# xianlopez/optical_flow

Measured on AMD Instinct MI355X. Metric: image-pairs/sec training, 384x512 batch=8 per GPU, higher is better.
Workload: dtype fp32

## Files before the change

optical_flow_amd/csrc/conv_f32.hip:

```cpp
#include "common.h"
#include "conv_dev.h"
#include "conv_narrow.h"

#include <algorithm>

namespace oflow {

template <int BM, int BN, int WAVES_M, int WAVES_N, int MODE>
__global__ __launch_bounds__(256, 2) void conv_gemm_f32(GemmArgs a) {
  constexpr int WM = BM / WAVES_M, WN = BN / WAVES_N;
  constexpr int TM = WM / 32, TN = WN / 32;
  static_assert(WAVES_M * WAVES_N == 4, "4 waves");
  static_assert(TM >= 1 && TN >= 1 && WM % 32 == 0 && WN % 32 == 0, "tile");
  constexpr bool A_KCONTIG = (MODE != MODE_WGRAD);
  constexpr int SA = BM + 4;
  constexpr int SB = BN + 4;
  constexpr int A_SLOTS = BM * BK / 4 / 256;
  constexpr int B_QUADS = BK * BN / 4;
  constexpr int B_SLOTS = (B_QUADS + 255) / 256;
  static_assert(A_SLOTS >= 1, "BM >= 64");

  static_assert(2 * BK * (SA + SB) >= 4 * 1024, "epilogue images fit LDS");
  __shared__ float smem[2 * BK * (SA + SB)];
  float (*As)[BK * SA] = reinterpret_cast<float (*)[BK * SA]>(smem);
// ... 2669 lines not shown
    }
  };
  auto store_halo = [&](int hb) {
#pragma unroll
    for (int k = 0; k < SW_HQ; ++k) {
      const int q = tid + NT * k;
      if (q >= SW_HH * SW_HX) continue;
      const int hy = q / SW_HX, hx = q - hy * SW_HX;
      float* dst = Hs[hb] + hy * 8 * SW_HC + (hx & 1) * SW_HC + (hx >> 1);
      dst[0] = hv[k].x;
      dst[2 * SW_HC] = hv[k].y;
      dst[4 * SW_HC] = hv[k].z;
      dst[6 * SW_HC] = hv[k].w;
    }
  };

  f32x4 acc[2][4];
#pragma unroll
  for (int i = 0; i < 2; ++i)
#pragma unroll
    for (int j = 0; j < 4; ++j)
#pragma unroll
      for (int r = 0; r < 4; ++r) acc[i][j][r] = 0.f;
  const int l16 = lane & 15, kg = lane >> 4;
  int a_off[2];
#pragma unroll
  for (int mt = 0; mt < 2; ++mt) {
    const int m = min(16 * (2 * wave + mt) + l16, 146);
    const int tap = m / 3, ci = m - 3 * tap, r = tap / 7, sc = tap - 7 * r;
    a_off[mt] = (r * 8 + ci * 2 + (sc & 1)) * SW_HC + 8 * kg + (sc >> 1);
  }

  if (nchunks > 0) {
    load_halo(t_begin);
    load_dz(0, dv[0], 0);
    if (nchunks > 1) load_dz(1, dv[1], 1);
    store_halo(0);
  }
  auto chunk = [&](int c, float* dvc, int set) {
    const int j = c % SW_TH, tl = c / SW_TH;
    const int buf = c & 1;
    if (j == 0 && tl + 1 < ntiles) load_halo(t_begin + tl + 1);
    if constexpr (FUSED) {
      if (tid < 256) form_dz(set, (j & 1) != 0, dvc);
    }
    store_dz(buf, dvc);
    __syncthreads();
    if (c + 2 < nchunks) load_dz(c + 2, dvc, set);
    if (j == 1 && tl + 1 < ntiles) store_halo((tl + 1) & 1);
    const float* hrow = Hs[tl & 1] + 2 * j * 8 * SW_HC;
    bf16x8 av[2][NP];
#pragma unroll
    for (int mt = 0; mt < 2; ++mt) {
      float v[8];
#pragma unroll
      for (int e = 0; e < 8; ++e) v[e] = hrow[a_off[mt] + e];
      if (NP == 1)
        av[mt][0] = __builtin_bit_cast(bf16x8, pack_bf16x8(make_float4(v[0], v[1], v[2], v[3]),
                                                           make_float4(v[4], v[5], v[6], v[7])));
      else
        split3x8(v, av[mt][0], av[mt][NP / 2], av[mt][NP - 1]);
    }
#pragma unroll
    for (int nt = 0; nt < 4; ++nt) {
      bf16x8 bv[NP];
#pragma unroll
      for (int p = 0; p < NP; ++p)
        bv[p] = __builtin_bit_cast(bf16x8, Ds[buf][(p * 4 + kg) * 64 + nt * 16 + l16]);
#pragma unroll
      for (int mt = 0; mt < 2; ++mt) {
        f32x4 x = acc[mt][nt];
        if (NP == 3) {
          x = __builtin_amdgcn_mfma_f32_16x16x32_bf16(av[mt][NP - 1], bv[0], x, 0, 0, 0);
          x = __builtin_amdgcn_mfma_f32_16x16x32_bf16(av[mt][0], bv[NP - 1], x, 0, 0, 0);
          x = __builtin_amdgcn_mfma_f32_16x16x32_bf16(av[mt][NP / 2], bv[NP / 2], x, 0, 0, 0);
          x = __builtin_amdgcn_mfma_f32_16x16x32_bf16(av[mt][NP / 2], bv[0], x, 0, 0, 0);
          x = __builtin_amdgcn_mfma_f32_16x16x32_bf16(av[mt][0], bv[NP / 2], x, 0, 0, 0);
        }
        acc[mt][nt] = __builtin_amdgcn_mfma_f32_16x16x32_bf16(av[mt][0], bv[0], x, 0, 0, 0);
      }
    }
  };
  for (int c = 0; c < nchunks; c += 2) {
    chunk(c, dv[0], 0);
    if (c + 1 < nchunks) chunk(c + 1, dv[1], 1);
  }

  float* slab = a.slab + (int64_t)split * a.split_stride;
#pragma unroll
  for (int mt = 0; mt < 2; ++mt)
#pragma unroll
    for (int rr = 0; rr < 4; ++rr) {
      const int m = 16 * (2 * wave + mt) + 4 * kg + rr;
      if (m >= 147) continue;
      const int tap = m / 3, ci = m - 3 * tap;
#pragma unroll
      for (int nt = 0; nt < 4; ++nt) {
        const int co = nt * 16 + l16;
        if (co < a.N) slab[(int64_t)(tap * 4 + ci) * a.slab_ld + co] = acc[mt][nt][rr];
      }
    }
  if (FUSED) {
    float* Cs = reinterpret_cast<float*>(&Ds[0][0]);
    __syncthreads();
    if (tid < 256) {
      Cs[d_kg * 64 + d_co] = f_st;
      Cs[256 + d_kg * 64 + d_co] = f_stz;
    }
    __syncthreads();
    if (tid < 128 && (tid & 63) < a.N) {
      const int o = (tid >> 6) * 256, cc = tid & 63;
      slab[(int64_t)(196 + (tid >> 6)) * a.slab_ld + cc] =
          (Cs[o + cc] + Cs[o + 64 + cc]) + (Cs[o + 128 + cc] + Cs[o + 192 + cc]);
    }
  } else if (a.colsum) {
    float* Cs = reinterpret_cast<float*>(&Ds[0][0]);
    __syncthreads();
    if (tid < 256) Cs[d_kg * 64 + d_co] = csum;
    __syncthreads();
    if (tid < 64 && tid < a.N)
      slab[(int64_t)196 * a.slab_ld + tid] = (Cs[tid] + Cs[64 + tid]) + (Cs[128 + tid] + Cs[192 + tid]);
  }
}

__global__ __launch_bounds__(256) void stem_bn_final(const float* __restrict__ slab, int splits,
                                                     int64_t split_stride, int ld, int c,
                                                     const float* __restrict__ gamma,
                                                     const float* __restrict__ var, float eps,
                                                     float* __restrict__ dgamma,
                                                     float* __restrict__ dbeta,
                                                     float* __restrict__ dbias, int accum) {
  __shared__ float red[2][4][64];
  const int co = threadIdx.x & 63, g = threadIdx.x >> 6;
  const int s0 = (int)((int64_t)g * splits / 4), s1 = (int)((int64_t)(g + 1) * splits / 4);
  float st = 0.f, stz = 0.f;
  if (co < c) {
    for (int sp = s0; sp < s1; ++sp) {
      st += slab[sp * split_stride + 196 * (int64_t)ld + co];
      stz += slab[sp * split_stride + 197 * (int64_t)ld + co];
    }
  }
  red[0][g][co] = st;
  red[1][g][co] = stz;
  __syncthreads();
  if (g != 0 || co >= c) return;
  st = (red[0][0][co] + red[0][1][co]) + (red[0][2][co] + red[0][3][co]);
  stz = (red[1][0][co] + red[1][1][co]) + (red[1][2][co] + red[1][3][co]);
  const float db = st * gamma[co] * rsqrtf(var[co] + eps);
  if (dbeta) dbeta[co] = accum ? dbeta[co] + st : st;
  if (dgamma) dgamma[co] = accum ? dgamma[co] + stz : stz;
  if (dbias) dbias[co] = accum ? dbias[co] + db : db;
}

template <int WAVES_CI, int WAVES_CO, int WAVES_R, int XH>
__global__ __launch_bounds__(64 * WAVES_CI * WAVES_CO * WAVES_R, 1) void conv_wgrad_tile_x3(GemmArgs a) {
  constexpr int NT = 64 * WAVES_CI * WAVES_CO * WAVES_R;
  static_assert(WAVES_R == 3, "one kernel row per wave group");
  constexpr int CIB = 32 * WAVES_CI, COB = 32 * WAVES_CO, KS = 3, HH = XH + KS - 1, NP = 3;
  constexpr int XQ = HH * KS * 2 * (CIB / 4), XS = (XQ + NT - 1) / NT;
  constexpr int PL = KS * HH * CIB * 2;
  __shared__ uint4 Xs[NP * PL];

  auto xrow = [](int ci) { return ci ^ ((ci >> 2) & 2); };
  auto xoct = [](int ci) { return (ci >> 4) & 1; };
  const int tid = threadIdx.x;
  const int lane = tid & 63;
  const int wave = __builtin_amdgcn_readfirstlane(tid >> 6);
  const int wgid = xcd_remap(blockIdx.x, gridDim.x);
  const int split = wgid / a.tiles_total;
  const int tile = wgid - split * a.tiles_total;
  const int tile_co = tile % a.n_tiles;
  const int tile_ci = tile / a.n_tiles;
  const int ci0 = tile_ci * CIB, co0 = tile_co * COB;
  const int t_begin = split * a.k_per_split;
  const int t_end = min(a.K, t_begin + a.k_per_split);
  const int steps = max(0, t_end - t_begin);
  const int tiles_x = (a.wo + TT_W - 1) / TT_W, tiles_y = (a.ho + XH - 1) / XH;
  const rsrc_t rx = make_rsrc(a.A, a.a_bytes);
  const rsrc_t rd = make_rsrc(a.B, a.b_bytes);
  const int wr = wave / (WAVES_CI * WAVES_CO);
  const int wci0 = ((wave / WAVES_CO) % WAVES_CI) * 32;
  const int wco0 = (wave % WAVES_CO) * 32;
  const int lrow = lane & 31, lk = lane >> 5;
  const bool do_colsum = a.colsum && tile_ci == 0 && wci0 == 0 && wr == 0;

  const int xcq = tid % (CIB / 4);
  const bool xc_ok = ci0 + 4 * xcq < a.kc;
  float4 xv[XS][8];
  auto load_x = [&](int t) {
    const int b = t / (tiles_x * tiles_y);
    const int trem = t - b * tiles_x * tiles_y;
    const int oy0 = (trem / tiles_x) * XH, ox0 = (trem % tiles_x) * TT_W;
    const int iy0 = oy0 - a.pt, ix00 = ox0 - a.pl;
#pragma unroll
    for (int j = 0; j < XS; ++j) {
      const int q = tid + NT * j;
      const int r2 = q / (CIB / 4);
      const int half = r2 & 1, s = (r2 >> 1) % KS, hy = (r2 >> 1) / KS;
      const int iy = iy0 + hy;
      const bool rok = q < XQ && xc_ok && (unsigned)iy < (unsigned)a.h;
      const int ix0 = ix00 + 8 * half + s;
      const int base = ((b * a.h + iy) * a.w + ix0) * a.lda + ci0 + 4 * xcq;
#pragma unroll
      for (int e = 0; e < 8; ++e) {
        const bool ok = rok && (unsigned)(ix0 + e) < (unsigned)a.w;
        xv[j][e] = bload4(rx, ok ? (uint32_t)((base + e * a.lda) * 4) : kOOB);
      }
    }
  };
  auto store_x = [&]() {
#pragma unroll
    for (int j = 0; j < XS; ++j) {
      const int q = tid + NT * j;
      if (q < XQ) {
        const int r2 = q / (CIB / 4);
        const int half = r2 & 1, s = (r2 >> 1) % KS, hy = (r2 >> 1) / KS;
        const int ci = 4 * xcq;
        uint4* blk = &Xs[(s * HH + hy) * CIB * 2];
#pragma unroll
        for (int c = 0; c < 4; ++c) {
          float v8[8];
#pragma unroll
          for (int e = 0; e < 8; ++e) v8[e] = (&xv[j][e].x)[c];
          bf16x8 h, m, l;
          split3x8(v8, h, m, l);
          const int idx = xrow(ci + c) * 2 + (half ^ xoct(ci + c));
          blk[idx] = __builtin_bit_cast(uint4, h);
          blk[PL + idx] = __builtin_bit_cast(uint4, m);
          blk[2 * PL + idx] = __builtin_bit_cast(uint4, l);
        }
      }
    }
  };
  const int co = co0 + wco0 + lrow;
  const bool co_ok = co < a.nb;
  const uint32_t dy_lane = (uint32_t)((8 * lk * a.ldb + co) * 4);
  const bool dy_co_full = co0 + COB <= a.nb;
  auto load_dy = [&](float (&dv)[8], int t, int kk) {
    const int b = t / (tiles_x * tiles_y);
    const int trem = t - b * tiles_x * tiles_y;
    const int oy = (trem / tiles_x) * XH + kk, ox0 = (trem % tiles_x) * TT_W;
    if (dy_co_full && oy < a.ho && ox0 + TT_W <= a.wo) {
      const int so = ((b * a.ho + oy) * a.wo + ox0) * a.ldb * 4;
#pragma unroll
      for (int e = 0; e < 8; ++e)
        dv[e] = __builtin_bit_cast(float, __builtin_amdgcn_raw_buffer_load_b32(
                                              rd, dy_lane + e * a.ldb * 4, so, 0));
      return;
    }
    const int ox = ox0 + 8 * lk;
    const bool rok = co_ok && oy < a.ho;
    const int base = ((b * a.ho + oy) * a.wo + ox) * a.ldb + co;
#pragma unroll
    for (int e = 0; e < 8; ++e) {
      const bool ok = rok && ox + e < a.wo;
      dv[e] = bload1(rd, ok ? (uint32_t)((base + e * a.ldb) * 4) : kOOB);
    }
  };

  f32x16 acc[KS];
#pragma unroll
  for (int t = 0; t < KS; ++t)
#pragma unroll
    for (int r = 0; r < 16; ++r) acc[t][r] = 0.f;
  const int a_base = xrow(wci0 + lrow) * 2 + (lk ^ xoct(wci0 + lrow));
  float colacc = 0.f;
  float dcur[8], dnext[8];

  if (steps > 0) {
    load_x(t_begin);
    load_dy(dcur, t_begin, 0);
    store_x();
  }
  __syncthreads();
  for (int i = 0; i < steps; ++i) {
    const int t = t_begin + i;
    const bool more = i + 1 < steps;
    if (more) load_x(t + 1);
#pragma unroll
    for (int kk = 0; kk < XH; ++kk) {
      if (kk + 1 < XH) load_dy(dnext, t, kk + 1);
      else if (more) load_dy(dnext, t + 1, 0);
      __builtin_amdgcn_sched_barrier(0);
      bf16x8 bh, bm, bl;
      split3x8(dcur, bh, bm, bl);
      if (do_colsum) {
#pragma unroll
        for (int e = 0; e < 8; ++e) colacc += dcur[e];
      }
      bf16x8 fa[2][NP];
      auto load_a = [&](bf16x8 (&f)[NP], int s) {
        const int xa = (s * HH + kk + wr) * CIB * 2 + a_base;
#pragma unroll
        for (int p = 0; p < NP; ++p) f[p] = __builtin_bit_cast(bf16x8, Xs[p * PL + xa]);
      };
      load_a(fa[0], 0);
#pragma unroll
      for (int s = 0; s < KS; ++s) {
          if (s + 1 < KS) load_a(fa[(s + 1) & 1], s + 1);
          __builtin_amdgcn_sched_barrier(0);
          const bf16x8 ah = fa[s & 1][0], am = fa[s & 1][1], al = fa[s & 1][2];
          f32x16 x = acc[s];
          x = __builtin_amdgcn_mfma_f32_32x32x16_bf16(al, bh, x, 0, 0, 0);
          x = __builtin_amdgcn_mfma_f32_32x32x16_bf16(ah, bl, x, 0, 0, 0);
          x = __builtin_amdgcn_mfma_f32_32x32x16_bf16(am, bm, x, 0, 0, 0);
          x = __builtin_amdgcn_mfma_f32_32x32x16_bf16(am, bh, x, 0, 0, 0);
          x = __builtin_amdgcn_mfma_f32_32x32x16_bf16(ah, bm, x, 0, 0, 0);
          acc[s] = __builtin_amdgcn_mfma_f32_32x32x16_bf16(ah, bh, x, 0, 0, 0);
          __builtin_amdgcn_sched_barrier(0);
      }
#pragma unroll
      for (int e = 0; e < 8; ++e) dcur[e] = dnext[e];
    }
    __syncthreads();
    if (more) store_x();
    __syncthreads();
  }

  float* S = a.slab + (int64_t)split * a.split_stride;
  if (do_colsum) {
    const float v = colacc + __shfl_xor(colacc, 32);
    if (lk == 0 && co < a.N) S[(int64_t)a.M * a.slab_ld + co] = v;
  }
  if (co < a.N) {
#pragma unroll
    for (int s = 0; s < KS; ++s)
#pragma unroll
      for (int r = 0; r < 16; ++r) {
        const int ci = ci0 + wci0 + (r & 3) + 8 * (r >> 2) + 4 * lk;
        if (ci < a.kc) S[((int64_t)(wr * KS + s) * a.kc + ci) * a.slab_ld + co] = acc[s][r];
      }
  }
}

__device__ __forceinline__ int wgx3b_slot(int ci, int oct) {
  return (ci >> 3) * 16 + ((2 * (ci & 7) + oct) ^ (((ci >> 3) & 3) << 1));
}

template <int CIB>
__device__ __forceinline__ int wgx3b_sw(int hx) {
  return ((hx >> 3) & 1) | (CIB == 64 ? ((hx >> 1) & 1) << 1 : 0);
}

template <int WAVES_CI, int WAVES_CO, int XH, int MI, int NP, int STG>
__device__ __forceinline__ void wgrad_x3b_body(const GemmArgs& a) {
  constexpr int NJ = 2 / MI;
  static_assert(MI * NJ == 2, "18 accumulator tiles per wave");
  static_assert(NP == 1 || NP == 3, "planes");
  static_assert(STG == 0 || STG == 1, "staging: three shifted copies / one pixel-major image");
  constexpr int NT = 64 * WAVES_CI * WAVES_CO;
  constexpr int CIB = 16 * MI * WAVES_CI, COB = 16 * NJ * WAVES_CO, KS = 3, HH = XH + KS - 1;
  static_assert(XH % 2 == 0 && (CIB == 32 || CIB == 64), "k-steps of 2 tile rows; wgx3b_sw");
  constexpr int HW = TT_W + KS - 1;
  constexpr int XQ = STG ? HH * HW * (CIB / 4) : HH * KS * 2 * (CIB / 4), XS = (XQ + NT - 1) / NT;
  constexpr int RB = CIB * 2;
  constexpr int PL = KS * HH * RB;
  constexpr int PXB = CIB * 2;
  constexpr int PLB = HH * HW * PXB, IMGB = NP * PLB;
  constexpr int LDSB = STG ? 2 * IMGB : NP * PL * 16;
  static_assert(NT / 64 * 512 * 4 <= LDSB && LDSB % 16 == 0, "epilogue images fit LDS");
  __shared__ uint4 Xs[LDSB / 16];
  char* const xlds = reinterpret_cast<char*>(Xs);

  const int tid = threadIdx.x;
  const int lane = tid & 63;
  const int wave = __builtin_amdgcn_readfirstlane(tid >> 6);
  const int wgid = xcd_remap(blockIdx.x, gridDim.x);
  const int split = wgid / a.tiles_total;
  const int tile = wgid - split * a.tiles_total;
  const int tile_co = tile % a.n_tiles;
  const int tile_ci = tile / a.n_tiles;
  const int ci0 = tile_ci * CIB, co0 = tile_co * COB;
  const int t_begin = split * a.k_per_split;
  const int t_end = min(a.K, t_begin + a.k_per_split);
  const int steps = max(0, t_end - t_begin);
  const int tiles_x = (a.wo + TT_W - 1) / TT_W, tiles_y = (a.ho + XH - 1) / XH;
  const rsrc_t rx = make_rsrc(a.A, a.a_bytes);
  const rsrc_t rd = make_rsrc(a.B, a.b_bytes);
  const int wci0 = (wave / WAVES_CO) * 16 * MI;
  const int wco0 = (wave % WAVES_CO) * 16 * NJ;
  const int l16 = lane & 15, lq = lane >> 4;

  const int xcq = tid % (CIB / 4);
  const bool xc_ok = ci0 + 4 * xcq < a.kc;
  constexpr int XE = STG ? 1 : 8;
  float4 xv[XS][XE];
  auto load_x = [&](int t) {
    const int b = t / (tiles_x * tiles_y);
    const int trem = t - b * tiles_x * tiles_y;
    const int oy0 = (trem / tiles_x) * XH, ox0 = (trem % tiles_x) * TT_W;
    const int iy0 = oy0 - a.pt, ix00 = ox0 - a.pl;
#pragma unroll
    for (int j = 0; j < XS; ++j) {
      const int q = tid + NT * j;
      if constexpr (STG == 1) {
        const int hp = q / (CIB / 4);
        const int hy = hp / HW, hx = hp - hy * HW;
        const int iy = iy0 + hy, ix = ix00 + hx;
        const bool ok = q < XQ && xc_ok && (unsigned)iy < (unsigned)a.h &&
                        (unsigned)ix < (unsigned)a.w;
        const int base = ((b * a.h + iy) * a.w + ix) * a.lda + ci0 + 4 * xcq;
        xv[j][0] = bload4(rx, ok ? (uint32_t)(base * 4) : kOOB);
      } else {
        const int r2 = q / (CIB / 4);
        const int half = r2 & 1, s = (r2 >> 1) % KS, hy = (r2 >> 1) / KS;
        const int iy = iy0 + hy;
        const bool rok = q < XQ && xc_ok && (unsigned)iy < (unsigned)a.h;
        const int ix0 = ix00 + 8 * half + s;
        const int base = ((b * a.h + iy) * a.w + ix0) * a.lda + ci0 + 4 * xcq;
#pragma unroll
        for (int e = 0; e < 8; ++e) {
          const bool ok = rok && (unsigned)(ix0 + e) < (unsigned)a.w;
          xv[j][e] = bload4(rx, ok ? (uint32_t)((base + e * a.lda) * 4) : kOOB);
        }
      }
    }
  };
  auto store_x = [&](int j, int buf) {
    const int q = tid + NT * j;
    if (XQ % NT == 0 || q < XQ) {
      if constexpr (STG == 1) {
        const int hp = q / (CIB / 4);
        const int hx = hp % HW;
        char* dst = xlds + buf * IMGB + hp * PXB + (((xcq >> 2) ^ wgx3b_sw<CIB>(hx)) << 5) +
                    8 * (xcq & 3);
        if constexpr (NP == 1) {
          *reinterpret_cast<uint2*>(dst) = pack_bf16x4(xv[j][0]);
        } else {
          uint2 h, m, l;
          split3x4(xv[j][0], h, m, l);
          *reinterpret_cast<uint2*>(dst) = h;
          *reinterpret_cast<uint2*>(dst + PLB) = m;
          *reinterpret_cast<uint2*>(dst + 2 * PLB) = l;
        }
      } else {
        const int r2 = q / (CIB / 4);
        const int half = r2 & 1, s = (r2 >> 1) % KS, hy = (r2 >> 1) / KS;
        uint4* blk = &Xs[(s * HH + hy) * RB];
#pragma unroll
        for (int c = 0; c < 4; ++c) {
          float v8[8];
#pragma unroll
          for (int e = 0; e < 8; ++e) v8[e] = (&xv[j][e].x)[c];
          const int idx = wgx3b_slot(4 * xcq + c, half);
          if constexpr (NP == 1) {
            blk[idx] = pack_bf16x8(make_float4(v8[0], v8[1], v8[2], v8[3]),
                                   make_float4(v8[4], v8[5], v8[6], v8[7]));
          } else {
            bf16x8 h, m, l;
            split3x8(v8, h, m, l);
            blk[idx] = __builtin_bit_cast(uint4, h);
            blk[PL + idx] = __builtin_bit_cast(uint4, m);
            blk[2 * PL + idx] = __builtin_bit_cast(uint4, l);
          }
        }
      }
    }
  };
  auto store_x_all = [&](int buf) {
#pragma unroll
    for (int j = 0; j < XS; ++j) store_x(j, buf);
  };
  int co[NJ];
  bool co_ok[NJ];
#pragma unroll
  for (int j = 0; j < NJ; ++j) {
    co[j] = co0 + wco0 + 16 * j + l16;
    co_ok[j] = co[j] < a.nb;
  }
  const int prow = lq >> 1, pcol = 8 * (lq & 1);
  const bool dy_co_full = co0 + COB <= a.nb;
  const uint32_t dy_lane = (uint32_t)(((prow * a.wo + pcol) * a.ldb + co0 + wco0 + l16) * 4);
  auto load_dy = [&](float (&dv)[NJ][8], int t, int kk) {
    const int b = t / (tiles_x * tiles_y);
    const int trem = t - b * tiles_x * tiles_y;
    const int oyr = (trem / tiles_x) * XH + 2 * kk, ox0 = (trem % tiles_x) * TT_W;
    if (dy_co_full && oyr + 1 < a.ho && ox0 + TT_W <= a.wo) {
      const int so = ((b * a.ho + oyr) * a.wo + ox0) * a.ldb * 4;
#pragma unroll
      for (int j = 0; j < NJ; ++j)
#pragma unroll
        for (int e = 0; e < 8; ++e)
          dv[j][e] = __builtin_bit_cast(float, __builtin_amdgcn_raw_buffer_load_b32(
                                                   rd, dy_lane + (e * a.ldb + 16 * j) * 4, so, 0));
      return;
    }
    const int oy = oyr + prow, ox = ox0 + pcol;
    const bool rok = oy < a.ho;
#pragma unroll
    for (int j = 0; j < NJ; ++j) {
      const int base = ((b * a.ho + oy) * a.wo + ox) * a.ldb + co[j];
#pragma unroll
      for (int e = 0; e < 8; ++e) {
        const bool ok = rok && co_ok[j] && ox + e < a.wo;
// ... 1535 lines not shown
  return with_cfg(T[cfg], cfg);
}

bool wgt_ok(const of_conv_desc* d, bool bf16) {
  if (!tile_ok(d)) return false;
  if (bf16) return true;
  const int64_t npix = (int64_t)d->n * d->ho * d->wo;
  return d->cout == 64 || (d->cout % 128 == 0 && npix <= 8 * 96 * 128);
}
int wgt_cfg(const of_conv_desc* d) { return d->cout > 64 ? 0 : 2; }
void wgt_blocks(const of_conv_desc* d, int& cib, int& cob) {
  cib = wgt_cfg(d) == 0 ? 32 : 64;
  cob = wgt_cfg(d) == 0 ? 128 : 64;
}

int wgx3_cfg(const of_conv_desc* d) {
  if (!tile_ok(d)) return -1;
  if (d->cout == 64) return d->cin_p % 64 == 0 || !g_wgx3_c4 ? 2 : 4;
  return d->cout % 128 == 0 ? 0 : d->cout == 96 ? 1 : d->cout == 32 ? 3 : -1;
}
bool wgx3_ok(const of_conv_desc* d) { return wgx3_cfg(d) >= 0; }
void wgx3_blocks(const of_conv_desc* d, int& cib, int& cob) {
  const int c = wgx3_cfg(d);
  cib = c == 2 || c == 3 ? 64 : 32;
  cob = c == 0 ? 128 : c == 1 ? 96 : c == 2 || c == 4 ? 64 : 32;
}

static int g_stem_wg = 1;
bool stem_wg_ok(const of_conv_desc* d) { return g_stem_wg && stem_x3_ok(d) && d->cin == 3; }
int stem_wg_tiles(const of_conv_desc* d) {
  return d->n * (int)cdiv(d->ho, SW_TH) * (int)cdiv(d->wo, SW_TW);
}

static int g_wgrad_wgs = 4;
static int g_x3_direct = 1;
static int g_bnp_b16 = 0;

static int g_gemm_b16 = 6;
static int g_wgt_pf = 1;

enum class Fam { narrow, gemm_f32, gemm_bf16, gemm_x3, gemm_b16, tile_bf16, tile_x3, tile_b16,
                 tile_ws, stem };
enum class WFam { narrow, stem, tile_x3, tile_b16, gemm_x3, gemm_b16, tile, gemm_bf16, gemm_f32 };

Fam gemm_family(int prec, int mode) {
  if (!prec) return Fam::gemm_f32;
  if (prec == 2) return Fam::gemm_x3;
  return (g_gemm_b16 & (mode == MODE_FWD ? 1 : 2)) ? Fam::gemm_b16 : Fam::gemm_bf16;
}
Fam tile_family(const of_conv_desc* d, int prec, int mode, bool bnp = false) {
  if (prec == 2) return Fam::tile_x3;
  if (ws_ok(d, mode)) return Fam::tile_ws;
  return g_tile_b16 == 1 || (bnp && g_bnp_b16) ? Fam::tile_b16 : Fam::tile_bf16;
}
Fam fwd_family(const of_conv_desc* d, int prec, bool plain, bool stem_kernel = true) {
  if (!prec) return narrow_ok(d) && plain ? Fam::narrow : Fam::gemm_f32;
  if (tile_ok(d)) return tile_family(d, prec, MODE_FWD);
  if (stem_kernel && (prec == 2 || g_stem_bf16) && g_stem_x3 && stem_x3_ok(d)) return Fam::stem;
  return gemm_family(prec, MODE_FWD);
}
Fam dgrad_family(const of_conv_desc* d, int prec, bool bnp = false) {
  if (!prec) return narrow_ok(d) ? Fam::narrow : Fam::gemm_f32;
  return tile_ok(d) ? tile_family(d, prec, MODE_DGRAD, bnp) : gemm_family(prec, MODE_DGRAD);
}

GemmArgs plan_args(const of_conv_desc* d, const Geo& g, int mode, Fam f, bool in_place = false) {
  if (f == Fam::tile_bf16 || f == Fam::tile_x3 || f == Fam::tile_b16 || f == Fam::tile_ws)
    return tile_args(d, g, mode, f == Fam::tile_x3, f == Fam::tile_b16, f == Fam::tile_ws);
  const bool k16 = f != Fam::gemm_f32 && f != Fam::narrow;
  GemmArgs a = mode == MODE_FWD ? fwd_args(d, g, k16) : dgrad_args(d, g, k16, in_place);
  if (f == Fam::gemm_x3 || f == Fam::gemm_b16) gemm_x3_plan(a);
  return a;
}

template <int MODE>
int launch_family(Fam f, const GemmArgs& a, hipStream_t s, double flops) {
  switch (f) {
    case Fam::tile_x3: return launch<MODE>(tile_x3_launch<MODE>(a), a, s, flops);
    case Fam::tile_ws:
      return launch<MODE>(with_cfg(tile_ws_launch(a, MODE), kind(KIND_TILE_WS, MODE, 0)), a, s, flops);
    case Fam::tile_b16: return launch<MODE>(tile_b16_launch<MODE>(a), a, s, flops);
    case Fam::tile_bf16: return launch<MODE>(tile_bf16_launch<MODE>(a), a, s, flops);
    case Fam::gemm_x3: return launch<MODE>(gemm_x3_launch<MODE>(a), a, s, flops);
    case Fam::gemm_b16: return launch<MODE>(gemm_x3_launch<MODE, 1>(a), a, s, flops);
    case Fam::gemm_bf16: return launch<MODE>(gemm_bf16_launch<MODE>(a), a, s, flops);
    case Fam::gemm_f32: return launch<MODE>(gemm_f32_launch<MODE>(a), a, s, flops);
    default: return fail(OF_EINVAL, "conv: no GEMM launch for this family");
  }
}

WFam wgrad_family(const of_conv_desc* d, int prec) {
  const bool bf16 = prec == 1;
  if (narrow_ok(d)) return WFam::narrow;
  if (stem_wg_ok(d) && (!bf16 || g_stem_bf16)) return WFam::stem;
  if (prec == 2 && wgx3_ok(d)) return WFam::tile_x3;
  if (bf16 && g_wgrad_b16 && wgx3_ok(d)) return WFam::tile_b16;
  if (prec == 2 && g_wgx3_gemm) return WFam::gemm_x3;
  if (bf16 && (g_gemm_b16 & 4) && !tile_ok(d)) return WFam::gemm_b16;
  if (wgt_ok(d, bf16)) return WFam::tile;
  return bf16 ? WFam::gemm_bf16 : WFam::gemm_f32;
}

void wgrad_tiles(GemmArgs& a, const of_conv_desc* d, const Geo& g, bool x3) {
  int cib, cob;
  x3 ? wgx3_blocks(d, cib, cob) : wgt_blocks(d, cib, cob);
  a.K = d->n * (int)cdiv(d->ho, x3 ? wgx3_rows(wgx3_cfg(d)) : TT_H) * (int)cdiv(d->wo, TT_W);
  a.n_tiles = (int)cdiv(d->cout, cob);
  a.tiles_total = (int)cdiv(g.cin_p, cib) * a.n_tiles;
}

WgradPlan wgrad_plan(const of_conv_desc* d, int prec) {
  Geo g = geo(d);
  const WFam f = wgrad_family(d, prec);
  WgradPlan p;
  p.M = g.taps * g.cin_p;
  p.ldc = g.cout_p;
  p.split_stride = (int64_t)(p.M + 1) * p.ldc;
  auto slice = [&p](int units, int splits, int step = 1) {
    p.k_per_split = (int)round_up(cdiv(units, std::max(1, splits)), step);
    p.splits = (int)cdiv(units, p.k_per_split);
    return p;
  };
  if (f == WFam::stem)
    return slice(stem_wg_tiles(d), std::min(stem_wg_tiles(d), SW_WGS_PER_CU * device_cus()));
  if (f == WFam::tile_x3 || f == WFam::tile_b16 || f == WFam::tile) {
    GemmArgs t{};
    wgrad_tiles(t, d, g, f != WFam::tile);
    const int splits = std::min(t.K, device_cus() / t.tiles_total);
    return slice(t.K, f == WFam::tile ? splits : std::min(splits, t.K / g_wgx3_min_tiles));
  }
  const int K = d->n * d->ho * d->wo;
  if (f == WFam::gemm_x3 || f == WFam::gemm_b16) {
    const int tiles = (int)(cdiv(p.M, 128) * cdiv(d->cout, d->cout > 64 ? 128 : 64));
    const int splits = std::max(1, (f == WFam::gemm_b16 ? 2 : 1) * device_cus() / tiles);
    return slice(K, std::min(splits, (int)std::max<int64_t>(1, cdiv(K, 8 * BKH))), BKH);
  }
  const int bk = prec == 1 ? BKH : BK;
  const int tiles = (int)(cdiv(p.M, pick_bm(d->cout)) * cdiv(d->cout, pick_bn(d->cout)));
  const int splits = std::max(1, (g_wgrad_wgs * device_cus()) / tiles);
  return slice(K, std::min(splits, (int)std::max<int64_t>(1, cdiv(K, 8 * bk))), bk);
}
size_t wgrad_workspace(const of_conv_desc* d, int prec) {
  if (validate(d) != OF_OK) return 0;
  if (narrow_ok(d)) return narrow_wgrad_ws(d);
  const WgradPlan p = wgrad_plan(d, prec);
  return (size_t)p.splits * p.split_stride * sizeof(float);
}

template <int NP, bool FUSED = false>
constexpr Launch wgrad_stem_rec() {
  return {conv_wgrad_stem_x3<NP, FUSED>, SW_NT, NP == 1 ? KIND_STEM_WG_B16 : KIND_STEM_WG_X3,
          FUSED ? "conv_wgrad_stem_x3 fused" : "conv_wgrad_stem_x3"};
}
template <int CI, int CO, int R, int XH>
constexpr Launch wgrad_tile_x3_rec() {
  return {conv_wgrad_tile_x3<CI, CO, R, XH>, 64 * CI * CO * R, kind(KIND_TILE_X3, MODE_WGRAD, 0),
          "conv_wgrad_tile_x3"};
}
template <int STAGE, int CI, int CO, int XH, int MI = 1>
constexpr Launch wgrad_x3b_rec() {
  return {STAGE ? conv_wgrad_tile_x3b<CI, CO, XH, MI> : conv_wgrad_tile_x3b_c3<CI, CO, XH, MI>,
          64 * CI * CO, KIND_WGRAD_X3B, "conv_wgrad_tile_x3"};
}
template <int STAGE, int CI, int CO, int XH>
constexpr Launch wgrad_b16_rec() {
  return {STAGE ? conv_wgrad_tile_b16<CI, CO, XH> : conv_wgrad_tile_b16_c3<CI, CO, XH>,
          64 * CI * CO, KIND_WGRAD_B16, "conv_wgrad_tile_b16"};
}
template <int CI, int CO, int PF = 1>
constexpr Launch wgrad_tile_bf16_rec() {
  return {conv_wgrad_tile_bf16<CI, CO, PF>, 256, kind(KIND_TILE_BF16, MODE_WGRAD, 0), "conv_wgrad_tile"};
}
template <int CI, int CO>
constexpr Launch wgrad_tile_f32_rec() {
  return {conv_wgrad_tile_f32<CI, CO>, 256, kind(KIND_TILE_F32, MODE_WGRAD, 0), "conv_wgrad_tile"};
}

Launch wgrad_tile_x3_launch(int cfg) {
  static const Launch B[2][2][5] = {
      {{wgrad_x3b_rec<0, 2, 4, 8>(), wgrad_x3b_rec<0, 2, 3, 8>(), wgrad_x3b_rec<0, 4, 2, 4>(),
        wgrad_x3b_rec<0, 4, 1, 4>(), wgrad_x3b_rec<0, 2, 2, 8>()},
       {wgrad_x3b_rec<0, 1, 8, 8, 2>(), wgrad_x3b_rec<0, 1, 6, 8, 2>(), wgrad_x3b_rec<0, 2, 4, 4, 2>(),
        wgrad_x3b_rec<0, 2, 2, 4, 2>(), wgrad_x3b_rec<0, 1, 4, 8, 2>()}},
      {{wgrad_x3b_rec<1, 2, 4, 8>(), wgrad_x3b_rec<1, 2, 3, 8>(), wgrad_x3b_rec<1, 4, 2, 4>(),
        wgrad_x3b_rec<1, 4, 1, 4>(), wgrad_x3b_rec<1, 2, 2, 8>()},
       {wgrad_x3b_rec<1, 1, 8, 8, 2>(), wgrad_x3b_rec<1, 1, 6, 8, 2>(), wgrad_x3b_rec<1, 2, 4, 4, 2>(),
        wgrad_x3b_rec<1, 2, 2, 4, 2>(), wgrad_x3b_rec<1, 1, 4, 8, 2>()}}};
  static const Launch T[4] = {wgrad_tile_x3_rec<1, 4, 3, 8>(), wgrad_tile_x3_rec<1, 3, 3, 8>(),
                              wgrad_tile_x3_rec<2, 2, 3, 4>(), wgrad_tile_x3_rec<2, 1, 3, 4>()};
  const bool x3b = g_wgx3b == 2 || (g_wgx3b == 1 && cfg == 0) || cfg == 4;
  return with_cfg(x3b ? B[g_wgx3b_stage][g_wgx3b_mi - 1][cfg] : T[cfg], cfg);
}
Launch wgrad_tile_b16_launch(int cfg) {
  static const Launch T[2][5] = {
      {wgrad_b16_rec<0, 2, 4, 8>(), wgrad_b16_rec<0, 2, 3, 8>(), wgrad_b16_rec<0, 4, 2, 4>(),
       wgrad_b16_rec<0, 4, 1, 4>(), wgrad_b16_rec<0, 2, 2, 8>()},
      {wgrad_b16_rec<1, 2, 4, 8>(), wgrad_b16_rec<1, 2, 3, 8>(), wgrad_b16_rec<1, 4, 2, 4>(),
       wgrad_b16_rec<1, 4, 1, 4>(), wgrad_b16_rec<1, 2, 2, 8>()}};
  return with_cfg(T[g_wgx3b_stage][cfg], cfg);
}
Launch wgrad_tile_launch(int cfg, bool bf16) {
  static const Launch T16[2][2] = {{wgrad_tile_bf16_rec<1, 4, 0>(), wgrad_tile_bf16_rec<2, 2, 0>()},
                                   {wgrad_tile_bf16_rec<1, 4>(), wgrad_tile_bf16_rec<2, 2>()}};
  static const Launch T32[2] = {wgrad_tile_f32_rec<1, 4>(), wgrad_tile_f32_rec<2, 2>()};
  return with_cfg(bf16 ? T16[g_wgt_pf != 0][cfg / 2] : T32[cfg / 2], cfg);
}

}
}

using namespace oflow;

extern "C" {

int64_t of_conv_wfwd_elems(const of_conv_desc* d) {
  if (validate(d) != OF_OK) return -1;
  Geo g = geo(d);
  return (int64_t)g.kf * g.nf;
}

int64_t of_conv_wbwd_elems(const of_conv_desc* d) {
  if (validate(d) != OF_OK) return -1;
  Geo g = geo(d);
  return g.kd * g.nd;
}

int64_t of_conv_wfwd16_elems(const of_conv_desc* d) {
  if (validate(d) != OF_OK) return -1;
  Geo g = geo(d);
  return (int64_t)g.cout_p * g.kf16;
}

int64_t of_conv_wbwd16_elems(const of_conv_desc* d) {
  if (validate(d) != OF_OK) return -1;
  Geo g = geo(d);
  return g.kd16 * g.nd;
}

static PackEntry pack_entry(const of_conv_desc* d, const float* w, void* wf, void* wd,
                            int bf16) {
  const Geo g = geo(d);
  PackEntry E{};
  E.w = w;
  E.wf = static_cast<float*>(wf);
  E.wd = static_cast<float*>(wd);
  E.taps = g.taps;
  E.kw = d->kw;
  E.cin = d->cin;
  E.cout = d->cout;
  E.cin_p = g.cin_p;
  E.cout_p = g.cout_p;
  E.kf = g.kf;
  E.nf = g.nf;
  E.nd = g.nd;
  E.bf16 = bf16;
  E.kf16 = g.kf16;
  E.kd16 = g.kd16;
  E.pg = g.pg;
  return E;
}

static int64_t pack_work(const of_conv_desc* d, int bf16) {
  const Geo g = geo(d);
  return bf16 ? (int64_t)g.cout_p * g.kf16 + g.kd16 * g.nd : (int64_t)g.kf * g.nf + g.kd * g.nd;
}

static int64_t pack_work_many(const of_conv_desc* d, int bf16) {
  const Geo g = geo(d);
  return bf16 ? g.kd16 * g.nd : (int64_t)g.kf * g.nf + g.kd * g.nd;
}
static int64_t pack_tiles16(const of_conv_desc* d, int bf16) {
  const Geo g = geo(d);
  return bf16 ? cdiv(g.cout_p, PK_TN) * cdiv(g.kf16, PK_TK) : 0;
}

int of_conv_pack_weights_bf16(const of_conv_desc* d, const float* w_hwio, void* w16_fwd,
                              void* w16_bwd, void* stream) {
  int st = validate(d);
  if (st) return st;
  OF_CHECK_ARG(w_hwio && w16_fwd && w16_bwd, "pack bf16: NULL pointer");
  const int64_t total = pack_work(d, 1);
  OF_CHECK_ARG(total < INT32_MAX, "pack: layer too large");
  const int blocks = (int)std::min<int64_t>(cdiv(total, 256), 4096);
  hipLaunchKernelGGL(pack_one_kernel, dim3(blocks), dim3(256), 0, as_stream(stream),
                     pack_entry(d, w_hwio, w16_fwd, w16_bwd, 1), total);
  return check_launch("pack_bf16");
}

int of_conv_pack_weights(const of_conv_desc* d, const float* w_hwio, float* w_fwd,
                         float* w_bwd, void* stream) {
  int st = validate(d);
  if (st) return st;
  OF_CHECK_ARG(w_hwio && w_fwd, "pack: NULL pointer");
  Geo g = geo(d);
  hipStream_t s = as_stream(stream);
  {
    const int64_t total = (int64_t)g.kf * g.nf;
    const int blocks = (int)std::min<int64_t>(cdiv(total, 256), 4096);
    hipLaunchKernelGGL(pack_fwd_kernel, dim3(blocks), dim3(256), 0, s, w_hwio, g.taps, d->cin,
                       d->cout, g.cin_p, g.kf, g.nf, w_fwd);
    if ((st = check_launch("pack_fwd"))) return st;
  }
  if (w_bwd) {
    const int64_t total = g.kd * g.nd;
    const int blocks = (int)std::min<int64_t>(cdiv(total, 256), 4096);
    hipLaunchKernelGGL(pack_bwd_kernel, dim3(blocks), dim3(256), 0, s, w_hwio, g.pg, d->kw,
                       d->cin, d->cout, g.cout_p, g.nd, w_bwd);
    if ((st = check_launch("pack_bwd"))) return st;
  }
  return OF_OK;
}

int of_set_tuning(int key, int value) {
  if (key == 8 && value >= 0 && value <= 2) { g_stem_x3 = value; return OF_OK; }
  if (key == 7 && (value == 0 || value == 1)) { g_warp_win = value; return OF_OK; }
  if (key == 9 && value >= 0 && value <= 7) { g_corr_blk = value; return OF_OK; }
  if (key == 19 && (value == 0 || value == 1)) { g_corr_ty8 = value; return OF_OK; }
  if (key == 10 && value >= 1 && value <= 16) { g_wgrad_wgs = value; return OF_OK; }
  if (key == 11 && (value == 0 || value == 1)) { g_wgx3_c4 = value; return OF_OK; }
  if (key == 1 && value >= 1 && value <= 16) { g_split_wgs = value; return OF_OK; }
  if (key == 2 && value >= 2 && value <= 64) { g_split_min_chunks = value; return OF_OK; }
  if (key == 3 && (value == 0 || value == 1)) { g_vec_ep = value; return OF_OK; }
  if (key == 4 && value >= 0 && value <= 2) { g_wgx3b = value; return OF_OK; }
  if (key == 5 && (value == 1 || value == 2)) { g_wgx3b_mi = value; return OF_OK; }
  if (key == 6 && (value == 0 || value == 1)) { g_wgx3_gemm = value; return OF_OK; }
  if (key == 12 && value >= 0 && value <= 3) { g_tile_b16 = value; return OF_OK; }
  if (key == 13 && (value == 0 || value == 1)) { g_wgrad_b16 = value; return OF_OK; }
  if (key == 14 && (value == 0 || value == 1)) { g_stem_wg = value; return OF_OK; }
  if (key == 15 && (value == 0 || value == 1)) { g_stem_bf16 = value; return OF_OK; }
  if (key == 16 && value >= 0 && value <= 7) { g_gemm_b16 = value; return OF_OK; }
  if (key == 18 && (value == 0 || value == 1)) { g_tall16_dgrad = value; return OF_OK; }
  if (key == 17 && (value == 0 || value == 1)) { g_wgt_pf = value; return OF_OK; }
  if (key == 20 && (value == 0 || value == 1)) { g_tile16_pf = value; return OF_OK; }
  if (key == 21 && value >= 0 && value <= 3) { g_b16i_abl = value; return OF_OK; }
  if (key == 22 && (value == 0 || value == 1)) { g_b16i_direct = value; return OF_OK; }
  if (key == 23 && value >= 0 && value <= 3) { g_x3_direct = value; return OF_OK; }
  if (key == 24 && value >= 0 && value <= 2) { g_b16i_persist = value; return OF_OK; }
  if (key == 25 && value >= 0 && value <= 1000) { g_x3t_ep = value; return OF_OK; }
  if (key == 26 && value >= 0 && value <= 1000) { g_x3g_ep = value; return OF_OK; }
  if (key == 27 && value >= 0 && value <= 100000) { g_x3_small_bn = value; return OF_OK; }
  if (key == 28 && value >= 0 && value <= 64) { g_det_rmax = value; return OF_OK; }
  if (key == 29 && value >= 0 && value <= 4) { g_wgr_lanes = value; return OF_OK; }
  if (key == 30 && value >= 0 && value <= 2) { g_gx3_ring = value; return OF_OK; }
  if (key == 31 && value >= -1 && value <= 8) { g_stem_persist = value; return OF_OK; }
// ... 638 lines not shown
```

Before: 659.0.

## Stage wgrad x3 input as single pixel-major image with double-buffered LDS

Adds a staging mode to the conv_wgrad_tile_x3 kernel. Input is loaded once per pixel into a swizzled pixel-major LDS image instead of three shifted copies, and A fragments are read with transposing loads. The LDS is double-buffered, and stores for the next tile are spread across the kk loop, which removes the second barrier per step. Each LDS buffer is smaller and global loads drop, but the kernel now needs two image buffers and more address arithmetic. The mode is chosen by the existing g_wgx3b_stage flag.

```diff
diff --git a/optical_flow_amd/csrc/conv_f32.hip b/optical_flow_amd/csrc/conv_f32.hip
--- a/optical_flow_amd/csrc/conv_f32.hip
+++ b/optical_flow_amd/csrc/conv_f32.hip
@@ -2845,14 +2845,27 @@
   if (dbias) dbias[co] = accum ? dbias[co] + db : db;
 }
 
-template <int WAVES_CI, int WAVES_CO, int WAVES_R, int XH>
-__global__ __launch_bounds__(64 * WAVES_CI * WAVES_CO * WAVES_R, 1) void conv_wgrad_tile_x3(GemmArgs a) {
+template <int CIB>
+__device__ __forceinline__ int wgx3b_sw(int hx) {
+  return ((hx >> 3) & 1) | (CIB == 64 ? ((hx >> 1) & 1) << 1 : 0);
+}
+
+template <int WAVES_CI, int WAVES_CO, int WAVES_R, int XH, int STG>
+__device__ __forceinline__ void wgrad_x3_body(const GemmArgs& a) {
   constexpr int NT = 64 * WAVES_CI * WAVES_CO * WAVES_R;
   static_assert(WAVES_R == 3, "one kernel row per wave group");
+  static_assert(STG == 0 || STG == 1, "staging: three shifted copies / one pixel-major image");
   constexpr int CIB = 32 * WAVES_CI, COB = 32 * WAVES_CO, KS = 3, HH = XH + KS - 1, NP = 3;
-  constexpr int XQ = HH * KS * 2 * (CIB / 4), XS = (XQ + NT - 1) / NT;
+  static_assert(CIB == 32 || CIB == 64, "wgx3b_sw");
+  constexpr int HW = TT_W + KS - 1;
+  constexpr int XQ = STG ? HH * HW * (CIB / 4) : HH * KS * 2 * (CIB / 4), XS = (XQ + NT - 1) / NT;
+  static_assert(NT % (CIB / 4) == 0, "a thread keeps its channel quad in every slot");
   constexpr int PL = KS * HH * CIB * 2;
-  __shared__ uint4 Xs[NP * PL];
+  constexpr int PXB = CIB * 2;
+  constexpr int PLB = HH * HW * PXB, IMGB = NP * PLB;
+  constexpr int LDSB = STG ? 2 * IMGB : NP * PL * 16;
+  __shared__ uint4 Xs[LDSB / 16];
+  char* const xlds = reinterpret_cast<char*>(Xs);
 
   auto xrow = [](int ci) { return ci ^ ((ci >> 2) & 2); };
   auto xoct = [](int ci) { return (ci >> 4) & 1; };
@@ -2879,7 +2892,8 @@
 
   const int xcq = tid % (CIB / 4);
   const bool xc_ok = ci0 + 4 * xcq < a.kc;
-  float4 xv[XS][8];
+  constexpr int XE = STG ? 1 : 8;
+  float4 xv[XS][XE];
   auto load_x = [&](int t) {
     const int b = t / (tiles_x * tiles_y);
     const int trem = t - b * tiles_x * tiles_y;
@@ -2888,24 +2902,43 @@
 #pragma unroll
     for (int j = 0; j < XS; ++j) {
       const int q = tid + NT * j;
-      const int r2 = q / (CIB / 4);
-      const int half = r2 & 1, s = (r2 >> 1) % KS, hy = (r2 >> 1) / KS;
-      const int iy = iy0 + hy;
-      const bool rok = q < XQ && xc_ok && (unsigned)iy < (unsigned)a.h;
-      const int ix0 = ix00 + 8 * half + s;
-      const int base = ((b * a.h + iy) * a.w + ix0) * a.lda + ci0 + 4 * xcq;
-#pragma unroll
-      for (int e = 0; e < 8; ++e) {
-        const bool ok = rok && (unsigned)(ix0 + e) < (unsigned)a.w;
-        xv[j][e] = bload4(rx, ok ? (uint32_t)((base + e * a.lda) * 4) : kOOB);
+      if constexpr (STG == 1) {
+        const int hp = q / (CIB / 4);
+        const int hy = hp / HW, hx = hp - hy * HW;
+        const int iy = iy0 + hy, ix = ix00 + hx;
+        const bool ok = q < XQ && xc_ok && (unsigned)iy < (unsigned)a.h &&
+                        (unsigned)ix < (unsigned)a.w;
+        const int base = ((b * a.h + iy) * a.w + ix) * a.lda + ci0 + 4 * xcq;
+        xv[j][0] = bload4(rx, ok ? (uint32_t)(base * 4) : kOOB);
+      } else {
+        const int r2 = q / (CIB / 4);
+        const int half = r2 & 1, s = (r2 >> 1) % KS, hy = (r2 >> 1) / KS;
+        const int iy = iy0 + hy;
+        const bool rok = q < XQ && xc_ok && (unsigned)iy < (unsigned)a.h;
+        const int ix0 = ix00 + 8 * half + s;
+        const int base = ((b * a.h + iy) * a.w + ix0) * a.lda + ci0 + 4 * xcq;
+#pragma unroll
+        for (int e = 0; e < 8; ++e) {
+          const bool ok = rok && (unsigned)(ix0 + e) < (unsigned)a.w;
+          xv[j][e] = bload4(rx, ok ? (uint32_t)((base + e * a.lda) * 4) : kOOB);
+        }
       }
     }
   };
-  auto store_x = [&]() {
-#pragma unroll
-    for (int j = 0; j < XS; ++j) {
-      const int q = tid + NT * j;
-      if (q < XQ) {
+  auto store_x = [&](int j, int buf) {
+    const int q = tid + NT * j;
+    if (XQ % NT == 0 || q < XQ) {
+      if constexpr (STG == 1) {
+        const int hp = q / (CIB / 4);
+        const int hx = hp % HW;
+        char* dst = xlds + buf * IMGB + hp * PXB + (((xcq >> 2) ^ wgx3b_sw<CIB>(hx)) << 5) +
+                    8 * (xcq & 3);
+        uint2 h, m, l;
+        split3x4(xv[j][0], h, m, l);
+        *reinterpret_cast<uint2*>(dst) = h;
+        *reinterpret_cast<uint2*>(dst + PLB) = m;
+        *reinterpret_cast<uint2*>(dst + 2 * PLB) = l;
+      } else {
         const int r2 = q / (CIB / 4);
         const int half = r2 & 1, s = (r2 >> 1) % KS, hy = (r2 >> 1) / KS;
         const int ci = 4 * xcq;
@@ -2924,6 +2957,10 @@
         }
       }
     }
+  };
+  auto store_x_all = [&](int buf) {
+#pragma unroll
+    for (int j = 0; j < XS; ++j) store_x(j, buf);
   };
   const int co = co0 + wco0 + lrow;
   const bool co_ok = co < a.nb;
@@ -2957,19 +2994,38 @@
 #pragma unroll
     for (int r = 0; r < 16; ++r) acc[t][r] = 0.f;
   const int a_base = xrow(wci0 + lrow) * 2 + (lk ^ xoct(wci0 + lrow));
+  int a_tr[KS][2];
+  if constexpr (STG == 1) {
+#pragma unroll
+    for (int s = 0; s < KS; ++s)
+#pragma unroll
+      for (int h = 0; h < 2; ++h) {
+        const int hx = 8 * lk + s + 4 * h + ((lane >> 2) & 3);
+        a_tr[s][h] = (wr * HW + hx) * PXB +
+                     ((((wci0 >> 4) + ((lane >> 4) & 1)) ^ wgx3b_sw<CIB>(hx)) << 5) + 8 * (lane & 3);
+      }
+  }
   float colacc = 0.f;
   float dcur[8], dnext[8];
 
   if (steps > 0) {
     load_x(t_begin);
     load_dy(dcur, t_begin, 0);
-    store_x();
+    store_x_all(0);
   }
   __syncthreads();
   for (int i = 0; i < steps; ++i) {
     const int t = t_begin + i;
     const bool more = i + 1 < steps;
     if (more) load_x(t + 1);
+    const int buf = STG ? i & 1 : 0;
+    int a_cur[KS][2];
+    if constexpr (STG == 1) {
+#pragma unroll
+      for (int s = 0; s < KS; ++s)
+#pragma unroll
+        for (int h = 0; h < 2; ++h) a_cur[s][h] = a_tr[s][h] + buf * IMGB;
+    }
 #pragma unroll
     for (int kk = 0; kk < XH; ++kk) {
       if (kk + 1 < XH) load_dy(dnext, t, kk + 1);
@@ -2983,9 +3039,17 @@
       }
       bf16x8 fa[2][NP];
       auto load_a = [&](bf16x8 (&f)[NP], int s) {
-        const int xa = (s * HH + kk + wr) * CIB * 2 + a_base;
-#pragma unroll
-        for (int p = 0; p < NP; ++p) f[p] = __builtin_bit_cast(bf16x8, Xs[p * PL + xa]);
+        if constexpr (STG == 1) {
+#pragma unroll
+          for (int p = 0; p < NP; ++p) {
+            const int ro = p * PLB + kk * HW * PXB;
+            f[p] = tr_frag(xlds, a_cur[s][0] + ro, a_cur[s][1] + ro);
+          }
+        } else {
+          const int xa = (s * HH + kk + wr) * CIB * 2 + a_base;
+#pragma unroll
+          for (int p = 0; p < NP; ++p) f[p] = __builtin_bit_cast(bf16x8, Xs[p * PL + xa]);
+        }
       };
       load_a(fa[0], 0);
 #pragma unroll
@@ -3004,10 +3068,20 @@
       }
 #pragma unroll
       for (int e = 0; e < 8; ++e) dcur[e] = dnext[e];
+      if constexpr (STG == 1) {
+        if (more) {
+#pragma unroll
+          for (int j = 0; j < XS; ++j)
+            if (j * XH / XS == kk) store_x(j, buf ^ 1);
+        }
+        __builtin_amdgcn_sched_barrier(0);
+      }
     }
     __syncthreads();
-    if (more) store_x();
-    __syncthreads();
+    if constexpr (STG == 0) {
+      if (more) store_x_all(0);
+      __syncthreads();
+    }
   }
 
   float* S = a.slab + (int64_t)split * a.split_stride;
@@ -3026,13 +3100,17 @@
   }
 }
 
+template <int WAVES_CI, int WAVES_CO, int WAVES_R, int XH>
+__global__ __launch_bounds__(64 * WAVES_CI * WAVES_CO * WAVES_R, 1) void conv_wgrad_tile_x3(GemmArgs a) {
+  wgrad_x3_body<WAVES_CI, WAVES_CO, WAVES_R, XH, 1>(a);
+}
+template <int WAVES_CI, int WAVES_CO, int WAVES_R, int XH>
+__global__ __launch_bounds__(64 * WAVES_CI * WAVES_CO * WAVES_R, 1) void conv_wgrad_tile_x3_c3(GemmArgs a) {
+  wgrad_x3_body<WAVES_CI, WAVES_CO, WAVES_R, XH, 0>(a);
+}
+
 __device__ __forceinline__ int wgx3b_slot(int ci, int oct) {
   return (ci >> 3) * 16 + ((2 * (ci & 7) + oct) ^ (((ci >> 3) & 3) << 1));
-}
-
-template <int CIB>
-__device__ __forceinline__ int wgx3b_sw(int hx) {
-  return ((hx >> 3) & 1) | (CIB == 64 ? ((hx >> 1) & 1) << 1 : 0);
 }
 
 template <int WAVES_CI, int WAVES_CO, int XH, int MI, int NP, int STG>
@@ -4874,10 +4952,10 @@
   return {conv_wgrad_stem_x3<NP, FUSED>, SW_NT, NP == 1 ? KIND_STEM_WG_B16 : KIND_STEM_WG_X3,
           FUSED ? "conv_wgrad_stem_x3 fused" : "conv_wgrad_stem_x3"};
 }
-template <int CI, int CO, int R, int XH>
+template <int STAGE, int CI, int CO, int R, int XH>
 constexpr Launch wgrad_tile_x3_rec() {
-  return {conv_wgrad_tile_x3<CI, CO, R, XH>, 64 * CI * CO * R, kind(KIND_TILE_X3, MODE_WGRAD, 0),
-          "conv_wgrad_tile_x3"};
+  return {STAGE ? conv_wgrad_tile_x3<CI, CO, R, XH> : conv_wgrad_tile_x3_c3<CI, CO, R, XH>,
+          64 * CI * CO * R, kind(KIND_TILE_X3, MODE_WGRAD, 0), "conv_wgrad_tile_x3"};
 }
 template <int STAGE, int CI, int CO, int XH, int MI = 1>
 constexpr Launch wgrad_x3b_rec() {
@@ -4908,10 +4986,13 @@
         wgrad_x3b_rec<1, 4, 1, 4>(), wgrad_x3b_rec<1, 2, 2, 8>()},
        {wgrad_x3b_rec<1, 1, 8, 8, 2>(), wgrad_x3b_rec<1, 1, 6, 8, 2>(), wgrad_x3b_rec<1, 2, 4, 4, 2>(),
         wgrad_x3b_rec<1, 2, 2, 4, 2>(), wgrad_x3b_rec<1, 1, 4, 8, 2>()}}};
-  static const Launch T[4] = {wgrad_tile_x3_rec<1, 4, 3, 8>(), wgrad_tile_x3_rec<1, 3, 3, 8>(),
-                              wgrad_tile_x3_rec<2, 2, 3, 4>(), wgrad_tile_x3_rec<2, 1, 3, 4>()};
+  static const Launch T[2][4] = {
+      {wgrad_tile_x3_rec<0, 1, 4, 3, 8>(), wgrad_tile_x3_rec<0, 1, 3, 3, 8>(),
+       wgrad_tile_x3_rec<0, 2, 2, 3, 4>(), wgrad_tile_x3_rec<0, 2, 1, 3, 4>()},
+      {wgrad_tile_x3_rec<1, 1, 4, 3, 8>(), wgrad_tile_x3_rec<1, 1, 3, 3, 8>(),
+       wgrad_tile_x3_rec<1, 2, 2, 3, 4>(), wgrad_tile_x3_rec<1, 2, 1, 3, 4>()}};
   const bool x3b = g_wgx3b == 2 || (g_wgx3b == 1 && cfg == 0) || cfg == 4;
-  return with_cfg(x3b ? B[g_wgx3b_stage][g_wgx3b_mi - 1][cfg] : T[cfg], cfg);
+  return with_cfg(x3b ? B[g_wgx3b_stage][g_wgx3b_mi - 1][cfg] : T[g_wgx3b_stage][cfg], cfg);
 }
 Launch wgrad_tile_b16_launch(int cfg) {
   static const Launch T[2][5] = {
```

Result: faster. 667.4 (median of 6 runs) (+1.3%).
